# soedinglab/plass

Hardware: AMD Instinct MI355X
Metric: read-overlaps/s per assembly iteration (higher is better)
Workload: dtype u8/u64 (integer hash, byte compare; f32 ratios)

## Files before the change

plass_amd/csrc/kmermatch.hip:

```cpp
#include "common.hpp"
#include "device_utils.hpp"
#include "host_util.hpp"
#include "linepart.hpp"
#include "xxh64_u64.hpp"
#include <algorithm>
#include <memory>
#include <type_traits>
#include <cstdlib>
#include <climits>
#include <cstring>

namespace plasship {

#include "kmermatch_extract.hpp"
#include "kmermatch_group.hpp"
#include "kmermatch_repsort.hpp"
}
using namespace plasship;

namespace {

struct Timer {
    plasship_ctx *ctx; int slot;
    void start(int s) { slot = s; (void) hipEventRecord(ctx->ev[s], ctx->stream); }
// ... 58 lines not shown
    const uint64_t want = (lines + 4ull * (uint64_t) numCU - 1) / (4ull * (uint64_t) numCU);
    return (uint32_t) std::max<uint64_t>((uint64_t) nb * minFactor, std::min<uint64_t>((uint64_t) nb * 64, std::max<uint64_t>(want, 1)));
}
static LineGeo lineGeometry(uint64_t totalSlots, bool lng, int numCU, uint64_t slotsAll = 0, int W = 1) {
    LineGeo g;
    const int maxBits = lng ? 9 : 10;
    const int lw = ceilLog2((uint64_t) std::max(W, 1));
    const int totalBits = std::min(2 * maxBits, std::max(lw, std::max(0, ceilLog2(((slotsAll ? slotsAll : totalSlots) + 1535) / 1536))));
    g.b1 = totalBits <= maxBits ? totalBits : std::max((totalBits + 1) / 2, lw); g.b2 = totalBits - g.b1;
    g.nb1 = 1u << g.b1; g.nb2 = g.b2 ? 1u << g.b2 : 0u;
    g.totalLines = (totalSlots + RPL - 1) / RPL;
    g.lastValid = g.totalLines ? (uint32_t) (totalSlots - (g.totalLines - 1) * RPL) : (uint32_t) RPL;
    g.PL1 = pieceLinesFor(g.totalLines, g.nb1, numCU, 8);
    g.nP1 = (g.totalLines + g.PL1 - 1) / g.PL1;
    g.cap1 = std::max<uint64_t>(g.nP1 * ((uint64_t) g.PL1 + g.nb1), 1);
    if (g.nb2) {
        g.PL2 = 0xFFFFFFFFu; g.maxP2 = g.nb1; g.cap2 = g.cap1 + (uint64_t) g.nb1 * g.nb2;
    }
    return g;
}
static uint64_t repLevel1Cap(uint64_t nRec, uint64_t nSeg, uint32_t PL, uint32_t nb) {
    const uint64_t lines = (nRec + RPL - 1) / RPL + nSeg;
    return lines + (lines / PL + nSeg + 1) * (uint64_t) nb;
}

__global__ void arenaStartKernel(const uint32_t *__restrict__ lineBeg, uint32_t bpb, uint32_t gGrid, uint32_t nBuckets, uint64_t *__restrict__ arenaStart) {
    for (uint32_t j = blockIdx.x * blockDim.x + threadIdx.x; j < gGrid; j += gridDim.x * blockDim.x)
        arenaStart[j] = (uint64_t) lineBeg[std::min(j * bpb, nBuckets - 1)] * RPL;
}
__global__ void bigNeedKernel(const uint32_t *__restrict__ lineCnt, const uint32_t *__restrict__ unique, uint32_t nBuckets, uint64_t *__restrict__ need, uint32_t wordsPerEntry) {
    for (uint32_t b = blockIdx.x * blockDim.x + threadIdx.x; b < nBuckets; b += gridDim.x * blockDim.x) {
        const uint64_t c = (uint64_t) lineCnt[b] * RPL;
        uint64_t v = 0;
        if (unique[b] == AGG_NEEDS_SCRATCH) { uint64_t P = 1; while (P < c) P <<= 1; v = wordsPerEntry * P; }
        need[b] = v;
    }
}
__global__ void sumU32Kernel(const uint32_t *__restrict__ v, uint32_t n, unsigned long long *__restrict__ out) {
    unsigned long long s = 0;
    for (uint32_t i = blockIdx.x * blockDim.x + threadIdx.x; i < n; i += gridDim.x * blockDim.x) s += v[i];
    s = waveReduceSumU64(s);
    if (laneId() == 0 && s) atomicAdd(out, s);
}

template <class K> static int setDynLds(K k, size_t bytes) {
    PH_CHECK(hipFuncSetAttribute(reinterpret_cast<const void *>(k), hipFuncAttributeMaxDynamicSharedMemorySize, (int) bytes));
    return PLASSHIP_OK;
}
template <bool NUCL, bool LONG, int MODE, bool LIST, bool EXTRAS>
static int launchLinePart(plasship_ctx *ctx, const LinePartArgs &a, uint64_t nPiecesBound) {
    const size_t lds = linePartLdsBytes(a.nb, sizeof(Rec<LONG>), EXTRAS);
    const bool big = lds > 72 * 1024;
    const unsigned grid = (unsigned) std::max<uint64_t>(1, std::min<uint64_t>(nPiecesBound, (uint64_t) ctx->numCU * (big ? 1u : 2u)));
    if (big) {
        auto k = linePartKernel<NUCL, LONG, MODE, LIST, EXTRAS, 1024, 4, true>;
        const int rc = setDynLds(k, lds); if (rc) return rc;
        hipLaunchKernelGGL(k, dim3(grid), dim3(1024), lds, ctx->stream, a);
    } else {
        auto k = linePartKernel<NUCL, LONG, MODE, LIST, EXTRAS, 512, 4, true>;
        const int rc = setDynLds(k, lds); if (rc) return rc;
        hipLaunchKernelGGL(k, dim3(grid), dim3(512), lds, ctx->stream, a);
    }
    return PLASSHIP_OK;
}

static int buildLineLists(plasship_ctx *ctx, const uint32_t *dTags, uint64_t capLines, uint32_t nb, uint32_t *dCount, uint32_t *dStart, uint32_t *dCursor, uint32_t *dList) {
    hipStream_t st = ctx->stream;
    PH_CHECK(hipMemsetAsync(dCount, 0, (size_t) nb * 4, st));
    const unsigned g = (unsigned) std::max<uint64_t>(1, std::min<uint64_t>((capLines + 4095) / 4096, (uint64_t) ctx->numCU * 8));
    const unsigned gs = (unsigned) std::max<uint64_t>(1, std::min<uint64_t>((capLines + TS_CHUNK - 1) / TS_CHUNK, (uint64_t) ctx->numCU * 2));
    hipLaunchKernelGGL(tagHistKernel, dim3(g), dim3(256), 0, st, dTags, capLines, nb, dCount);
    hipLaunchKernelGGL(tagScanKernel, dim3(1), dim3(1024), 0, st, (const uint32_t *) dCount, nb, dStart, dCursor);
    hipLaunchKernelGGL(tagScatterKernel, dim3(gs), dim3(TS_BLOCK), 0, st, dTags, capLines, nb, dCursor, dList);
    return PLASSHIP_OK;
}

static bool shardOwnerFiltered(int W) { const int m = tuneInt("SHARD_EXTRACT", 0); return m == 2 || (m != 1 && W <= 4); }

constexpr int KM_RETRY_EARLY_OVERFLOW_CHECK = -1000;
struct LinesOut { void *triples = nullptr; uint64_t nTriples = 0, Nk = 0, Nm = 0; std::vector<int64_t> stalePos; uint32_t staleT = 0; float msSort1 = 0, msGroup = 0, msSort2 = 0, msPart = 0; int nPart = 1;
                  uint64_t exchangedRecordBytes = 0, exchangedTripleBytes = 0; };

constexpr uint64_t HALO_SLACK = 1u << 16;

template <bool NUCL, bool LONG, bool TRIPLES, bool ORDOUT = false>
static int repSortLines(plasship_ctx *ctx, const void *in, const std::vector<std::pair<uint64_t, uint64_t>> &segs, uint64_t nIn, uint32_t nReps, uint32_t repBase, uint32_t nTargets,
                        uint64_t slackTriples, const std::function<void()> &inputConsumed, DevBuf &dOut, uint64_t &nTriples, DevBuf *dRepStartOut) {
    constexpr bool PL = TRIPLES ? NUCL : LONG;
    typedef Rec<PL> R;
    typedef typename std::conditional<ORDOUT, TripleX, Triple>::type OutT;
    hipStream_t st = ctx->stream;
    const int numCU = ctx->numCU;
    const int maxBits = PL ? 9 : 10;
    const int idBits = std::max(1, ceilLog2((uint64_t) nTargets));
    const int repBits = std::max(1, ceilLog2((uint64_t) std::max<uint32_t>(nReps, 1)));
    const int wantBits = std::min(2 * maxBits, std::max(0, ceilLog2((nIn + 511) / 512)));
    const int allowedLocal = 62 - idBits - DiagPack<LONG>::BITS;
    const int sBits = std::max(std::min(wantBits, repBits), std::max(0, repBits - allowedLocal));
    if (sBits > 2 * maxBits) { setError("kmermatch: too many sequences for the packed rep-sort key"); return PLASSHIP_ERR_UNSUPPORTED; }
    const int s1 = sBits <= maxBits ? sBits : (sBits + 1) / 2, s2 = sBits - s1;
    const uint32_t nS1 = 1u << s1, nS2 = s2 ? 1u << s2 : 0u, nSort = 1u << sBits;
    std::vector<LinePiece> hp; uint64_t outLine = 0;
    {
        uint64_t totLines = 0; for (const auto &sg : segs) totLines += (sg.second + RPL - 1) / RPL;
        const uint32_t PLr1 = pieceLinesFor(totLines, nS1, numCU, 8);
        for (const auto &sg : segs) {
            const uint64_t cnt = sg.second, lines = (cnt + RPL - 1) / RPL;
            for (uint64_t l0 = 0; l0 < lines; l0 += PLr1) {
                LinePiece pc; pc.in0 = sg.first + l0; pc.nLines = (uint32_t) std::min<uint64_t>(PLr1, lines - l0);
                pc.lastValid = (l0 + pc.nLines == lines) ? (uint32_t) (cnt - (lines - 1) * RPL) : (uint32_t) RPL;
                pc.out0 = outLine; pc.outCap = pc.nLines + nS1; pc.tagBase = 0;
                outLine += pc.outCap; hp.push_back(pc);
            }
        }
    }
    const uint32_t PLr2 = s2 ? pieceLinesFor(std::max<uint64_t>(outLine, 1), nS2, numCU, 16) : 0;
    const uint64_t maxPR2 = s2 ? std::max<uint64_t>(outLine, 1) / PLr2 + nS1 + 1 : 0;
    const uint64_t capR1 = std::max<uint64_t>(outLine, 1), capR2 = s2 ? capR1 + maxPR2 * nS2 : 0;
    const uint32_t nPR1 = (uint32_t) hp.size();
    DevBuf dR1, dRTag1, dRList1, dRPieces, dRNP, dRCnt1, dRStart1, dRCur1, dR2, dRTag2, dRList2, dRPieces2, dRNP2, dRRegBeg, dRRegEnd, dRTot2, dSortBeg, dSortCnt;
    if (dR1.alloc(capR1 * RPL * sizeof(R)) != hipSuccess || dRTag1.alloc(capR1 * 4) != hipSuccess || dRList1.alloc(capR1 * 4) != hipSuccess || dRPieces.alloc(((size_t) nPR1 + 1) * sizeof(LinePiece)) != hipSuccess ||
        dRNP.alloc(4) != hipSuccess || dRCnt1.alloc(LP_MAXB * 4) != hipSuccess || dRStart1.alloc((LP_MAXB + 1) * 4) != hipSuccess || dRCur1.alloc(LP_MAXB * 4) != hipSuccess ||
        dSortBeg.alloc((size_t) nSort * 4) != hipSuccess || dSortCnt.alloc((size_t) nSort * 4) != hipSuccess) { setError("kmermatch: out of device memory for the rep sort"); return PLASSHIP_ERR_DEVICE; }
    void *hpPinned = nPR1 ? ctxPinnedTable(ctx, (size_t) nPR1 * sizeof(LinePiece)) : nullptr;
    if (hpPinned) memcpy(hpPinned, hp.data(), (size_t) nPR1 * sizeof(LinePiece));
    if (nPR1) PH_CHECK(hipMemcpyAsync(dRPieces.p, hpPinned ? hpPinned : (const void *) hp.data(), (size_t) nPR1 * sizeof(LinePiece), hipMemcpyHostToDevice, st));
    else PH_CHECK(hipMemsetAsync(dRTag1.p, 0xFF, capR1 * 4, st));
    PH_CHECK(hipMemcpyAsync(dRNP.p, &nPR1, 4, hipMemcpyHostToDevice, st));
    static const int directLines = [] { const char *e = getenv("PLASSHIP_DIRECT_LINES"); return e ? atoi(e) : 1; }();
    LineKey rkey; rkey.rangeBits = repBits; rkey.repBase = repBase; rkey.shift = s1 ? 64 - s1 : 63; rkey.scrambleBits = repBits;
    int rc;
    {
        LinePartArgs a; memset(&a, 0, sizeof(a));
        a.in = in; a.out = dR1.p; a.tags = dRTag1.as<uint32_t>(); a.pieces = dRPieces.as<LinePiece>(); a.nPieces = dRNP.as<uint32_t>(); a.nb = nS1; a.key = rkey;
        a.direct = directLines;
        rc = launchLinePart<NUCL, PL, KEY_RANGE, false, false>(ctx, a, std::max<uint32_t>(nPR1, 1)); if (rc) return rc;
    }
    if (nPR1 && !hpPinned) PH_CHECK(plasship::streamSync(st));
    rc = buildLineLists(ctx, dRTag1.as<uint32_t>(), capR1, nS1, dRCnt1.as<uint32_t>(), dRStart1.as<uint32_t>(), dRCur1.as<uint32_t>(), dRList1.as<uint32_t>()); if (rc) return rc;
    inputConsumed();
    const void *sortRecs = dR1.p; const uint32_t *sortList = dRList1.as<uint32_t>(); uint64_t sortCap = capR1;
    if (s2) {
        if (dR2.alloc(capR2 * RPL * sizeof(R)) != hipSuccess || dRTag2.alloc(capR2 * 4) != hipSuccess || dRList2.alloc(capR2 * 4) != hipSuccess || dRPieces2.alloc(((size_t) maxPR2 + 1) * sizeof(LinePiece)) != hipSuccess ||
            dRNP2.alloc(4) != hipSuccess || dRRegBeg.alloc(LP_MAXB * 8) != hipSuccess || dRRegEnd.alloc(LP_MAXB * 8) != hipSuccess || dRTot2.alloc(8) != hipSuccess) { setError("kmermatch: out of device memory for the rep sort"); return PLASSHIP_ERR_DEVICE; }
        hipLaunchKernelGGL(planListKernel, dim3(1), dim3(1024), 0, st, (const uint32_t *) dRStart1.as<uint32_t>(), nS1, PLr2, nS2, dRPieces2.as<LinePiece>(), dRNP2.as<uint32_t>(),
                           dRRegBeg.as<uint64_t>(), dRRegEnd.as<uint64_t>(), dRTot2.as<uint64_t>());
        LinePartArgs a; memset(&a, 0, sizeof(a));
        a.in = dR1.p; a.list = dRList1.as<uint32_t>(); a.out = dR2.p; a.tags = dRTag2.as<uint32_t>(); a.pieces = dRPieces2.as<LinePiece>(); a.nPieces = dRNP2.as<uint32_t>(); a.nb = nS2;
        a.direct = directLines;
        a.key = rkey; a.key.shift = 64 - s1 - s2;
        rc = launchLinePart<NUCL, PL, KEY_RANGE, true, false>(ctx, a, maxPR2); if (rc) return rc;
        hipLaunchKernelGGL(tagSortRegionKernel, dim3(std::min<uint32_t>(nS1, (uint32_t) numCU * 4)), dim3(512), 0, st, (const uint32_t *) dRTag2.as<uint32_t>(), (const uint64_t *) dRRegBeg.as<uint64_t>(),
                           (const uint64_t *) dRRegEnd.as<uint64_t>(), nS1, nS2, dRList2.as<uint32_t>(), dSortBeg.as<uint32_t>(), dSortCnt.as<uint32_t>());
        sortRecs = dR2.p; sortList = dRList2.as<uint32_t>(); sortCap = capR2;
    } else {
        hipLaunchKernelGGL(listRangesKernel, dim3(4), dim3(256), 0, st, (const uint32_t *) dRStart1.as<uint32_t>(), nS1, dSortBeg.as<uint32_t>(), dSortCnt.as<uint32_t>());
    }
    DevBuf dBigNeed, dBigOff, dBigScratch, dUnique, dScanTmp3, dSparse;
    const size_t scanTmp3Bytes = exclusiveScanTmpBytes((size_t) nSort + 2);
    if (dBigNeed.alloc(((size_t) nSort + 1) * 8) != hipSuccess || dBigOff.alloc(((size_t) nSort + 2) * 8) != hipSuccess || dUnique.alloc(((size_t) nSort + 1) * 4) != hipSuccess ||
        dScanTmp3.alloc(scanTmp3Bytes) != hipSuccess || dSparse.alloc(sortCap * RPL * sizeof(OutT)) != hipSuccess) {
        setError("kmermatch: out of device memory for the rep sort"); return PLASSHIP_ERR_DEVICE;
    }
    const AggLines aggLn{sortList, dSortBeg.as<uint32_t>(), dSortCnt.as<uint32_t>()};
    const unsigned aggGrid = std::min<uint32_t>(nSort, (uint32_t) numCU * (uint32_t) tuneInt("AGGSORT", 16));
    hipLaunchKernelGGL((aggSortKernel<NUCL, LONG, true, TRIPLES, ORDOUT>), dim3(aggGrid), dim3(LS_BLOCK), 0, st, sortRecs, dSparse.p, (const uint64_t *) nullptr, nSort,
                       (unsigned long long *) nullptr, (const uint64_t *) nullptr, dUnique.as<uint32_t>(), repBits - sBits, idBits, (uint64_t) repBase, aggLn, repBits);
    hipLaunchKernelGGL(bigNeedKernel, dim3(gridFor(nSort, 256, 1024)), dim3(256), 0, st, (const uint32_t *) dSortCnt.as<uint32_t>(), (const uint32_t *) dUnique.as<uint32_t>(), nSort, dBigNeed.as<uint64_t>(), NUCL ? 3u : 2u);
    if (exclusiveScanU64(st, dBigNeed.as<uint64_t>(), dBigOff.as<uint64_t>(), nSort, dScanTmp3.p, scanTmp3Bytes)) { setError("kmermatch: scan failed"); return PLASSHIP_ERR_DEVICE; }
    uint64_t bigTot = 0;
    PH_COPY_SYNC(st, &bigTot, dBigOff.as<uint64_t>() + nSort, 8, hipMemcpyDeviceToHost);
    PH_CHECK(hipGetLastError());
    if (bigTot) {
        if (dBigScratch.alloc(bigTot * 8) != hipSuccess) { setError("kmermatch: out of device memory for the rep sort"); return PLASSHIP_ERR_DEVICE; }
        hipLaunchKernelGGL((aggSortKernel<NUCL, LONG, true, TRIPLES, ORDOUT>), dim3(aggGrid), dim3(LS_BLOCK), 0, st, sortRecs, dSparse.p, (const uint64_t *) nullptr, nSort,
                           dBigScratch.as<unsigned long long>(), (const uint64_t *) dBigOff.as<uint64_t>(), dUnique.as<uint32_t>(), repBits - sBits, idBits, (uint64_t) repBase, aggLn, repBits);
    }
    DevBuf dRepCnt, dRepStartLocal, dScanTmp4;
    DevBuf &dRepStart = dRepStartOut ? *dRepStartOut : dRepStartLocal;
    const size_t scanTmp4Bytes = exclusiveScanTmpBytes((size_t) nReps + 2);
    if (dRepCnt.alloc(((size_t) nReps + 1) * 4) != hipSuccess || dRepStart.alloc(((size_t) nReps + 2) * 8) != hipSuccess ||
        dScanTmp4.alloc(scanTmp4Bytes) != hipSuccess) { setError("kmermatch: out of device memory for the rep sort"); return PLASSHIP_ERR_DEVICE; }
    PH_CHECK(hipMemsetAsync(dRepCnt.p, 0, ((size_t) nReps + 1) * 4, st));
    const unsigned runGrid = std::min<uint32_t>((nSort + 3) / 4, (uint32_t) numCU * 8);
    hipLaunchKernelGGL(repRunsKernel<OutT>, dim3(runGrid), dim3(256), 0, st, (const OutT *) dSparse.p, (const uint32_t *) dSortBeg.as<uint32_t>(),
                       (const uint32_t *) dUnique.as<uint32_t>(), nSort, repBase, dRepCnt.as<uint32_t>());
    if (exclusiveScanU32(st, dRepCnt.as<uint32_t>(), dRepStart.as<uint64_t>(), nReps, dScanTmp4.p, scanTmp4Bytes)) { setError("kmermatch: scan failed"); return PLASSHIP_ERR_DEVICE; }
    nTriples = 0;
    PH_COPY_SYNC(st, &nTriples, dRepStart.as<uint64_t>() + nReps, 8, hipMemcpyDeviceToHost);
    PH_CHECK(hipGetLastError());
    dR1.release(); dR2.release();
    if (dOut.alloc((std::max<uint64_t>(nTriples, 1) + slackTriples) * sizeof(OutT)) != hipSuccess) { setError("kmermatch: out of device memory for the sorted triples"); return PLASSHIP_ERR_DEVICE; }
    if (nTriples) hipLaunchKernelGGL(placeRunsKernel<OutT>, dim3(runGrid), dim3(256), 0, st, (const OutT *) dSparse.p, (const uint32_t *) dSortBeg.as<uint32_t>(), (const uint32_t *) dUnique.as<uint32_t>(), nSort,
                                     repBase, (const uint64_t *) dRepStart.as<uint64_t>(), (OutT *) dOut.p);
    PH_CHECK(hipGetLastError());
    return PLASSHIP_OK;
}

static void moveBuf(DevBuf &dst, DevBuf &src) { dst.release(); dst.p = src.p; dst.bytes = src.bytes; src.p = nullptr; src.bytes = 0; }

template <bool NUCL, bool LONG>
static int kmermatchLines(plasship_ctx *ctx, const plasship_seqdb *db, const plasship_kmermatch_params *par, const LineGeo &geo, uint64_t total,
                          DevBuf &dA, DevBuf &dB, const DevBuf &dSlotOff, const DevBuf &dKStats, const ExtractArgs &ea, int keyBits, LinesOut &res,
                          const uint32_t *dLateOverflow, bool filtered) {
    typedef Rec<LONG> R;
    hipStream_t st = ctx->stream;
    const uint32_t N = (uint32_t) db->n;
    const int numCU = ctx->numCU;
    const plasship_comm *cm = commOf(ctx);
    const int W = cm ? cm->world : 1, rk = cm ? cm->rank : 0;
    const bool exch = cm && !filtered;
    const int valueShift = std::max(0, keyBits - 11);
    PH_CHECK(hipEventRecord(ctx->ev[1], st));
    const uint32_t bLo = cm ? (uint32_t) ownedBegin(geo.nb1, rk, W) : 0u, bHi = cm ? (uint32_t) ownedBegin(geo.nb1, rk + 1, W) : geo.nb1;
    const uint32_t nbL = bHi - bLo;
    DevBuf dVHist, dMinKey, dTag1, dList1, dCnt1, dStart1, dCur1, dTag2, dList2, dPieces2, dNP2, dRegBeg, dRegEnd, dTot2, dFineBeg, dFineCnt;
    DevBuf dRx, dRxList, dRxSegs, dRxStart;
    const uint32_t nBuckets = geo.nb2 ? nbL * geo.nb2 : nbL;
    if (dVHist.alloc(VH_BINS * 4) != hipSuccess || dMinKey.alloc(8) != hipSuccess || dTag1.alloc(geo.cap1 * 4) != hipSuccess || dList1.alloc(geo.cap1 * 4) != hipSuccess ||
        dCnt1.alloc(LP_MAXB * 4) != hipSuccess || dStart1.alloc((LP_MAXB + 1) * 4) != hipSuccess || dCur1.alloc(LP_MAXB * 4) != hipSuccess ||
        dFineBeg.alloc((size_t) std::max<uint32_t>(nBuckets, 1) * 4) != hipSuccess || dFineCnt.alloc((size_t) std::max<uint32_t>(nBuckets, 1) * 4) != hipSuccess ||
        (geo.nb2 && (dPieces2.alloc((geo.maxP2 + 1) * sizeof(LinePiece)) != hipSuccess ||
                     dNP2.alloc(4) != hipSuccess || dRegBeg.alloc(LP_MAXB * 8) != hipSuccess || dRegEnd.alloc(LP_MAXB * 8) != hipSuccess || dTot2.alloc(8) != hipSuccess))) {
        setError("kmermatch: out of device memory for the line lists"); return PLASSHIP_ERR_DEVICE;
    }
    PH_CHECK(hipMemsetAsync(dVHist.p, 0, VH_BINS * 4, st));
    PH_CHECK(hipMemsetAsync(dMinKey.p, 0xFF, 8, st));
    if (geo.nP1 == 0) PH_CHECK(hipMemsetAsync(dTag1.p, 0xFF, geo.cap1 * 4, st));
    {
        LinePartArgs a; memset(&a, 0, sizeof(a));
        a.in = dA.p; a.out = dB.p; a.tags = dTag1.as<uint32_t>(); a.totalLines = geo.totalLines; a.lastValidAll = geo.lastValid; a.pieceLines = geo.PL1; a.nb = geo.nb1;
        a.key.shift = geo.b1 ? 64 - geo.b1 : 63; a.key.rangeBits = 0; a.key.repBase = 0;
        a.minKey = NUCL ? dMinKey.as<unsigned long long>() : nullptr; a.valueHist = dVHist.as<uint32_t>(); a.valueShift = valueShift;
        if (cm && filtered) { a.keepLo = bLo; a.keepHi = bHi; }
        PH_CHECK(hipEventRecord(ctx->ev[8], st));
        const int rc = launchLinePart<NUCL, LONG, KEY_HASH, false, true>(ctx, a, geo.nP1); if (rc) return rc;
        PH_CHECK(hipEventRecord(ctx->ev[9], st));
    }
    int rc = buildLineLists(ctx, dTag1.as<uint32_t>(), geo.cap1, geo.nb1, dCnt1.as<uint32_t>(), dStart1.as<uint32_t>(), dCur1.as<uint32_t>(), dList1.as<uint32_t>()); if (rc) return rc;
    void *l1Recs = dB.p; const uint32_t *l1List = dList1.as<uint32_t>(); const uint32_t *l1Start = dStart1.as<uint32_t>() + bLo; uint64_t l1Lines = geo.cap1;
    const uint32_t *l1Tags = dTag1.as<uint32_t>();
    uint64_t NkAll = 0;
    if (cm && filtered && NUCL) {
        uint64_t mk = 0; PH_COPY_SYNC(st, &mk, dMinKey.p, 8, hipMemcpyDeviceToHost);
        rc = commAllReduceMinU64(ctx, &mk, 1); if (rc) return rc;
        PH_COPY_SYNC(st, dMinKey.p, &mk, 8, hipMemcpyHostToDevice);
    }
    if (exch) {
        std::vector<uint32_t> hStart1(geo.nb1 + 1);
        PH_COPY_SYNC(st, hStart1.data(), dStart1.p, ((size_t) geo.nb1 + 1) * 4, hipMemcpyDeviceToHost);
        PH_CHECK(hipGetLastError());
        const uint64_t myLines = hStart1[geo.nb1];
        const uint64_t selfBeg = hStart1[ownedBegin(geo.nb1, rk, W)], selfEnd = hStart1[ownedBegin(geo.nb1, rk + 1, W)];
        const uint64_t selfLines = selfEnd - selfBeg, sendLines = myLines - selfLines;
        const uint32_t chunksPerLine = (uint32_t) (RPL * sizeof(R) / 16);
        auto gather = [&](uint64_t listFrom, uint64_t n, void *dst) {
            if (n) hipLaunchKernelGGL(gatherLinesKernel, dim3(gridFor(n * chunksPerLine, 256, (unsigned) numCU * 16)), dim3(256), 0, st, (const uint4 *) dB.p, (const uint32_t *) dList1.as<uint32_t>() + listFrom,
                                      n, chunksPerLine, (uint4 *) dst);
        };
        dA.release();
        if (dA.alloc(std::max<uint64_t>(sendLines, 1) * RPL * sizeof(R)) != hipSuccess) { setError("kmermatch: out of device memory for the send buffer"); return PLASSHIP_ERR_DEVICE; }
        gather(0, selfBeg, dA.p);
        gather(selfEnd, myLines - selfEnd, (char *) dA.p + selfBeg * RPL * sizeof(R));
        dTag1.release();
        std::vector<uint64_t> mine((size_t) geo.nb1 + 1), all(((size_t) geo.nb1 + 1) * (size_t) W);
        for (uint32_t j = 0; j < geo.nb1; j++) mine[j] = hStart1[j + 1] - hStart1[j];
        { unsigned long long ks[4] = {0, 0, 0, 0}; PH_COPY_SYNC(st, ks, dKStats.p, 32, hipMemcpyDeviceToHost); mine[geo.nb1] = ks[1] + ks[3]; }
        rc = commAllgatherHost(ctx, mine.data(), all.data(), mine.size() * 8); if (rc) return rc;
        std::vector<uint64_t> sendCount(W);
// ... 653 lines not shown
```

plass_amd/csrc/kmermatch_repsort.hpp:

```cpp
#pragma once

constexpr int LS_BLOCK = 256;
constexpr uint32_t AGG_CAP = 1024;
constexpr uint32_t AGG_HT = 2048;
constexpr uint32_t AGG_NEEDS_SCRATCH = 0xFFFFFFFFu;
template <bool LONG> struct DiagPack { static constexpr int BITS = LONG ? 22 : 16; static constexpr int64_t BIAS = LONG ? (1 << 21) : 32768; };
struct __attribute__((aligned(16))) Triple { uint32_t rep, target; int32_t diag; uint32_t cnt; };
struct __attribute__((aligned(8))) TripleX { uint32_t rep, target; int32_t diag; uint32_t cnt; uint64_t ord; };
static_assert(sizeof(TripleX) == sizeof(Rec<true>) && sizeof(Triple) == sizeof(Rec<false>), "triples travel through the line store as records");

struct AggLines { const uint32_t *list, *lineBeg, *lineCnt; };
__device__ __forceinline__ bool isSentinel(const Triple &t) { return t.rep == 0xFFFFFFFFu && t.target == 0xFFFFFFFFu; }
__device__ __forceinline__ bool isSentinel(const TripleX &t) { return t.rep == 0xFFFFFFFFu && t.target == 0xFFFFFFFFu; }
template <bool NUCL, bool LONG, bool LINES, bool TRIPLES = false, bool ORDOUT = false>
__global__ __launch_bounds__(LS_BLOCK) void aggSortKernel(const void *arr, void *outTriples, const uint64_t *__restrict__ bucketStart, uint32_t nBuckets,
                                                          unsigned long long *bigScratch, const uint64_t *__restrict__ bigOff,
                                                          uint32_t *__restrict__ uniqueCount, int localBits, int idBits, uint64_t repBase, AggLines ln, int scrambleBits) {
    static_assert(!ORDOUT || NUCL, "only nucleotide triples carry a strand");
    typedef typename std::conditional<TRIPLES, typename std::conditional<NUCL, TripleX, Triple>::type, Rec<LONG>>::type R;
    typedef typename std::conditional<ORDOUT, TripleX, Triple>::type O;
    __shared__ unsigned long long hKey[AGG_HT];
    __shared__ uint32_t hVal[AGG_HT];
    __shared__ unsigned long long hOrd[NUCL ? AGG_HT : 1];
    __shared__ unsigned long long lKey[AGG_CAP];
    __shared__ uint32_t lVal[AGG_CAP];
    __shared__ unsigned long long lOrd[NUCL ? AGG_CAP : 1];
    __shared__ uint32_t sCount;
    __shared__ uint32_t sDistinct, sOver;
    __shared__ uint32_t sWave[LS_BLOCK / 64];
    const R *g = reinterpret_cast<const R *>(arr);
    O *out = reinterpret_cast<O *>(outTriples);
    constexpr int DB = DiagPack<LONG>::BITS;
    for (uint32_t b = blockIdx.x; b < nBuckets; b += gridDim.x) {
        const uint64_t s0 = LINES ? (uint64_t) ln.lineBeg[b] * RPL : bucketStart[b];
        const uint64_t cnt = LINES ? (uint64_t) ln.lineCnt[b] * RPL : bucketStart[b + 1] - s0;
        const uint32_t lb = LINES ? ln.lineBeg[b] : 0u;
        auto recAt = [&](uint64_t i) -> R { if (LINES) return g[(uint64_t) ln.list[lb + (uint32_t) (i / RPL)] * RPL + (i % RPL)]; return g[s0 + i]; };
        if (cnt == 0) { if (threadIdx.x == 0) uniqueCount[b] = 0; continue; }
        const uint64_t bucketBase = (uint64_t) b << localBits;
        auto decode = [&](unsigned long long key, uint32_t val, unsigned long long ord) {
            O t;
            t.diag = (int32_t) ((int64_t) (key & ((1ULL << DB) - 1)) - DiagPack<LONG>::BIAS);
            const uint64_t k2 = key >> DB;
            t.target = (uint32_t) (k2 & ((1ULL << idBits) - 1));
            const uint64_t rp = (k2 >> idBits) + bucketBase;
            t.rep = (uint32_t) ((scrambleBits ? scrambleRep(rp, scrambleBits) : rp) + repBase);
            t.cnt = val;
            if constexpr (ORDOUT) t.ord = ord;
            return t;
        };
        auto packRec = [&](const R &r, uint32_t &val, unsigned long long &ord) {
            uint64_t rep, target; int64_t diag; ord = 0;
            if constexpr (TRIPLES) { rep = r.rep; target = r.target; diag = r.diag; val = r.cnt & 0x7FFFFFFFu; if constexpr (NUCL) ord = r.ord; }
            else { rep = (uint32_t) r.kmer; target = r.id; diag = r.pos; val = 1u; if constexpr (NUCL) ord = ordWordOf(r); }
            rep -= repBase;
            if (scrambleBits) rep = scrambleRep(rep, scrambleBits);
            return (unsigned long long) (((((rep - bucketBase) << idBits) | target) << DB) | (uint64_t) (diag + DiagPack<LONG>::BIAS));
        };
        auto clearTable = [&]() {
            for (uint32_t i = threadIdx.x; i < AGG_HT; i += LS_BLOCK) { hKey[i] = ~0ULL; hVal[i] = 0; if (NUCL) hOrd[i] = 0; }
            if (threadIdx.x == 0) sCount = 0;
            __syncthreads();
        };
        auto insert = [&](unsigned long long key, uint32_t val, unsigned long long ord) {
            uint32_t slot = (uint32_t) ((key * 0x9E3779B97F4A7C15ULL) >> 40) & (AGG_HT - 1);
            for (;;) {
                const unsigned long long prev = atomicCAS(&hKey[slot], ~0ULL, key);
                if (prev == ~0ULL || prev == key) break;
                slot = (slot + 1) & (AGG_HT - 1);
            }
            atomicAdd(&hVal[slot], val);
            if (NUCL) atomicMax(&hOrd[slot], ord);
        };
        auto extract = [&]() {
            for (uint32_t i = threadIdx.x; i < AGG_HT; i += LS_BLOCK) {
                const unsigned long long k = hKey[i];
                if (k != ~0ULL) {
                    const uint32_t o = atomicAdd(&sCount, 1u); lKey[o] = k;
                    if (NUCL) { const unsigned long long od = hOrd[i]; lOrd[o] = od; lVal[o] = hVal[i] | ((uint32_t) (od & 1ULL) << 31); }
                    else lVal[o] = hVal[i];
                }
            }
            __syncthreads();
            return sCount;
        };
        auto sortListAndWrite = [&](uint32_t U) {
            uint32_t P = 1; while (P < U) P <<= 1;
            for (uint32_t i = U + threadIdx.x; i < P; i += LS_BLOCK) { lKey[i] = ~0ULL; lVal[i] = 0; if (ORDOUT) lOrd[i] = 0; }
            __syncthreads();
            for (uint32_t kk = 2; kk <= P; kk <<= 1) {
                for (uint32_t j = kk >> 1; j > 0; j >>= 1) {
                    for (uint32_t t = threadIdx.x; t < (P >> 1); t += LS_BLOCK) {
                        const uint32_t i = ((t & ~(j - 1)) << 1) | (t & (j - 1));
                        const uint32_t l = i | j;
                        const unsigned long long x = lKey[i], y = lKey[l];
                        const bool up = (i & kk) == 0;
                        if ((x > y) == up) {
                            lKey[i] = y; lKey[l] = x; const uint32_t vx = lVal[i]; lVal[i] = lVal[l]; lVal[l] = vx;
                            if (ORDOUT) { const unsigned long long ox = lOrd[i]; lOrd[i] = lOrd[l]; lOrd[l] = ox; }
                        }
                    }
                    __syncthreads();
                }
            }
            for (uint32_t i = threadIdx.x; i < U; i += LS_BLOCK) out[s0 + i] = decode(lKey[i], lVal[i], ORDOUT ? lOrd[i] : 0ull);
            if (threadIdx.x == 0) uniqueCount[b] = U;
            __syncthreads();
        };
        if (bigScratch && uniqueCount[b] != AGG_NEEDS_SCRATCH) continue;
        bool done = false;
        if (!bigScratch && cnt <= (1ull << 22)) {
            clearTable();
            if (threadIdx.x == 0) { sDistinct = 0; sOver = 0; }
            __syncthreads();
            for (uint64_t i = threadIdx.x; i < cnt && !*(volatile uint32_t *) &sOver; i += LS_BLOCK) {
                const R r = recAt(i); if (LINES && isSentinel(r)) continue;
// ... 18 lines not shown
        if (!bigScratch) { if (threadIdx.x == 0) uniqueCount[b] = AGG_NEEDS_SCRATCH; continue; }
        {
            unsigned long long *pk = bigScratch + bigOff[b];
            uint64_t P0 = 1; while (P0 < cnt) P0 <<= 1;
            unsigned long long *pv = pk + P0, *po = pv + P0;
            uint64_t nPart = 0;
            for (uint64_t c0 = 0; c0 < cnt; c0 += AGG_CAP) {
                const uint64_t c1 = min(cnt, c0 + (uint64_t) AGG_CAP);
                clearTable();
                for (uint64_t i = c0 + threadIdx.x; i < c1; i += LS_BLOCK) { const R r = recAt(i); if (LINES && isSentinel(r)) continue; uint32_t v; unsigned long long od; const unsigned long long key = packRec(r, v, od); insert(key, v, od); }
                __syncthreads();
                const uint32_t U = extract();
                for (uint32_t i = threadIdx.x; i < U; i += LS_BLOCK) { pk[nPart + i] = lKey[i]; pv[nPart + i] = lVal[i] & 0x7FFFFFFFu; if (NUCL) po[nPart + i] = lOrd[i]; }
                nPart += U;
                __syncthreads();
            }
            bool fits = true;
            if (nPart <= (uint64_t) AGG_HT) {
                clearTable();
                for (uint64_t i = threadIdx.x; i < nPart; i += LS_BLOCK) insert(pk[i], (uint32_t) pv[i], NUCL ? po[i] : 0ull);
                __syncthreads();
                uint32_t mine = 0;
                for (uint32_t i = threadIdx.x; i < AGG_HT; i += LS_BLOCK) mine += (hKey[i] != ~0ULL) ? 1u : 0u;
                mine = (uint32_t) waveReduceSum((int) mine);
                if (laneId() == 0) sWave[threadIdx.x >> 6] = mine;
                __syncthreads();
                uint32_t tot = 0;
#pragma unroll
                for (int w = 0; w < LS_BLOCK / 64; w++) tot += sWave[w];
                __syncthreads();
                fits = tot <= AGG_CAP;
                if (fits) sortListAndWrite(extract());
            } else fits = false;
            if (!fits) {
                uint64_t P = 1; while (P < nPart) P <<= 1;
                for (uint64_t i = nPart + threadIdx.x; i < P; i += LS_BLOCK) { pk[i] = ~0ULL; pv[i] = 0; if (NUCL) po[i] = 0; }
                __syncthreads();
                for (uint64_t kk = 2; kk <= P; kk <<= 1) {
                    for (uint64_t j = kk >> 1; j > 0; j >>= 1) {
                        for (uint64_t t = threadIdx.x; t < (P >> 1); t += LS_BLOCK) {
                            const uint64_t i = ((t & ~(j - 1)) << 1) | (t & (j - 1));
                            const uint64_t l = i | j;
                            const unsigned long long x = pk[i], y = pk[l];
                            const bool up = (i & kk) == 0;
                            if ((x > y) == up) {
                                pk[i] = y; pk[l] = x; const unsigned long long vx = pv[i]; pv[i] = pv[l]; pv[l] = vx;
                                if (NUCL) { const unsigned long long ox = po[i]; po[i] = po[l]; po[l] = ox; }
                            }
                        }
                        __syncthreads();
                    }
                }
                uint32_t written = 0;
                for (uint64_t i0 = 0; i0 < nPart; i0 += LS_BLOCK) {
                    const uint64_t i = i0 + threadIdx.x;
                    bool head = false; O t; t.rep = t.target = t.cnt = 0; t.diag = 0;
                    if (i < nPart) {
                        const unsigned long long k = pk[i];
                        head = (i == 0) || (pk[i - 1] != k);
                        if (head) {
                            uint32_t c = 0; unsigned long long om = 0;
                            for (uint64_t j = i; j < nPart && pk[j] == k; j++) { c += (uint32_t) pv[j]; if (NUCL) om = max(om, po[j]); }
                            t = decode(k, c | ((uint32_t) (om & 1ULL) << 31), om);
                        }
                    }
                    const unsigned long long mk = __ballot(head);
                    const uint32_t wr = (uint32_t) __popcll(mk & ((1ULL << laneId()) - 1ULL));
                    if (laneId() == 0) sWave[threadIdx.x >> 6] = (uint32_t) __popcll(mk);
                    __syncthreads();
                    uint32_t woff = 0, tot = 0;
#pragma unroll
                    for (int w = 0; w < LS_BLOCK / 64; w++) { if (w < (int) (threadIdx.x >> 6)) woff += sWave[w]; tot += sWave[w]; }
                    if (head) out[s0 + written + woff + wr] = t;
                    written += tot;
                    __syncthreads();
                }
                if (threadIdx.x == 0) uniqueCount[b] = written;
                __syncthreads();
            }
        }
    }
}

template <class T>
__global__ __launch_bounds__(256) void repRunsKernel(const T *__restrict__ in, const uint32_t *__restrict__ lineBeg, const uint32_t *__restrict__ unique, uint32_t nBuckets,
                                                     uint32_t repBase, uint32_t *__restrict__ cnt) {
    for (uint32_t b = blockIdx.x * 4 + (threadIdx.x >> 6); b < nBuckets; b += gridDim.x * 4) {
        const uint64_t s0 = (uint64_t) lineBeg[b] * RPL; const uint32_t n = unique[b];
        for (uint32_t i0 = 0; i0 < n; i0 += 64) {
            const uint32_t i = i0 + laneId();
            const bool valid = i < n;
            const uint32_t rep = valid ? in[s0 + i].rep : 0xFFFFFFFFu;
            const uint32_t prevLane = __shfl_up(rep, 1, 64);
            const bool segHead = valid && (laneId() == 0 || prevLane != rep);
            const unsigned long long heads = __ballot(segHead), vmask = __ballot(valid);
            if (segHead) {
                const unsigned long long later = heads & ~((2ULL << laneId()) - 1ULL);
                const int end = later ? __ffsll((long long) later) - 1 : (int) __popcll(vmask);
                atomicAdd(&cnt[rep - repBase], (uint32_t) (end - laneId()));
            }
        }
    }
}
template <class T>
__global__ __launch_bounds__(256) void placeRunsKernel(const T *__restrict__ in, const uint32_t *__restrict__ lineBeg, const uint32_t *__restrict__ unique, uint32_t nBuckets,
                                                       uint32_t repBase, const uint64_t *__restrict__ start, T *__restrict__ out) {
    const int lane = laneId();
    for (uint32_t b = blockIdx.x * 4 + (threadIdx.x >> 6); b < nBuckets; b += gridDim.x * 4) {
        const uint64_t s0 = (uint64_t) lineBeg[b] * RPL; const uint32_t n = unique[b];
        uint32_t carryRep = 0xFFFFFFFFu, carryHead = 0;
        for (uint32_t i0 = 0; i0 < n; i0 += 64) {
            const uint32_t i = i0 + (uint32_t) lane;
            const bool valid = i < n;
            T t; t.rep = 0xFFFFFFFFu; t.target = 0; t.diag = 0; t.cnt = 0;
            if (valid) t = in[s0 + i];
            const uint32_t rep = t.rep;
            const uint32_t prevLane = __shfl_up(rep, 1, 64);
            const bool segHead = valid && (lane == 0 || prevLane != rep);
            const unsigned long long heads = __ballot(segHead), vmask = __ballot(valid);
            const unsigned long long below = heads & ((lane == 63) ? ~0ULL : ((2ULL << lane) - 1ULL));
            const int headLane = 63 - __clzll((long long) below);
            const uint32_t rep0 = (uint32_t) __shfl((int) rep, 0, 64);
            const uint32_t runHead = (headLane == 0 && rep0 == carryRep) ? carryHead : i0 + (uint32_t) headLane;
            if (valid) out[start[rep - repBase] + (uint64_t) (i - runHead)] = t;
            const int lastLane = (int) __popcll(vmask) - 1;
            carryRep = (uint32_t) __shfl((int) rep, lastLane, 64); carryHead = (uint32_t) __shfl((int) runHead, lastLane, 64);
        }
    }
}
__global__ void ownerBoundsKernel(const uint64_t *__restrict__ start, uint64_t n, int W, uint64_t *__restrict__ out) {
    for (int r = threadIdx.x; r <= W; r += blockDim.x) out[r] = start[((uint64_t) r * n + (uint64_t) W - 1) / (uint64_t) W];
}
__global__ __launch_bounds__(256) void gatherLinesKernel(const uint4 *__restrict__ in, const uint32_t *__restrict__ list, uint64_t nLines, uint32_t chunksPerLine, uint4 *__restrict__ out) {
    const uint64_t total = nLines * chunksPerLine;
    for (uint64_t i = (uint64_t) blockIdx.x * blockDim.x + threadIdx.x; i < total; i += (uint64_t) gridDim.x * blockDim.x)
        out[i] = in[(uint64_t) list[i / chunksPerLine] * chunksPerLine + (i % chunksPerLine)];
}
struct RxSeg { uint64_t src; uint32_t cnt, dst; };
__global__ __launch_bounds__(256) void rxListKernel(const RxSeg *__restrict__ segs, uint32_t nSegs, uint32_t *__restrict__ list) {
    for (uint32_t q = blockIdx.x; q < nSegs; q += gridDim.x) { const RxSeg g = segs[q]; for (uint32_t i = threadIdx.x; i < g.cnt; i += 256) list[g.dst + i] = (uint32_t) (g.src + i); }
}

template <bool NUCL>
__global__ __launch_bounds__(256) void reduceRunsKernel(const Triple *__restrict__ h, uint64_t n, uint64_t nScan, CandHit *__restrict__ tmpHits, uint32_t *__restrict__ emitW,
                                 uint32_t *__restrict__ perRep) {
    const int lane = threadIdx.x & 63;
    for (uint64_t i = (uint64_t) blockIdx.x * blockDim.x + threadIdx.x; i < n; i += (uint64_t) gridDim.x * blockDim.x) {
        const Triple r = h[i];
        bool head = (i == 0);
        if (!head) { const Triple q = h[i - 1]; head = (q.rep != r.rep) || (q.target != r.target); }
        uint32_t e = 0;
        CandHit c; c.target = 0; c.prefScore = 0; c.diag16 = 0; c.query = 0;
        if (head) {
            const uint32_t targetId = r.target;
            int32_t diagonal = r.diag, prevDiagonal = r.diag;
            uint64_t maxDiagonal = 0, diagonalCnt = 0, topScore = 0;
            int bestRev = NUCL ? ((r.cnt & 0x80000000u) == 0) : 0;
            for (uint64_t j = i; j < nScan; j++) {
                const Triple x = h[j];
                if (x.target != targetId) break;
                const uint64_t cc = x.cnt & 0x7FFFFFFFu;
                if (prevDiagonal == x.diag) diagonalCnt += cc; else diagonalCnt = cc;
                if (diagonalCnt >= maxDiagonal) { diagonal = x.diag; maxDiagonal = diagonalCnt; if (NUCL) bestRev = ((x.cnt & 0x80000000u) == 0); }
                prevDiagonal = x.diag; topScore += cc;
            }
            if (targetId != r.rep) {
                c.target = targetId; c.prefScore = bestRev ? -(int) topScore : (int) topScore;
                c.diag16 = (uint32_t) (uint16_t) diagonal; c.query = r.rep;
                e = 1;
            }
// ... 65 lines not shown
```

Before: 685.3 million.

## Add wave-per-bucket LDS hash aggregation with overflow list for rep sort

```diff
diff --git a/plass_amd/csrc/kmermatch.hip b/plass_amd/csrc/kmermatch.hip
--- a/plass_amd/csrc/kmermatch.hip
+++ b/plass_amd/csrc/kmermatch.hip
@@ -164,6 +164,29 @@
                   uint64_t exchangedRecordBytes = 0, exchangedTripleBytes = 0; };
 
 constexpr uint64_t HALO_SLACK = 1u << 16;
+
+static bool aggHistOn() { return getenv("PLASSHIP_DEBUG_AGGHIST") != nullptr; }
+static int aggHistRecord(hipStream_t st, const uint32_t *dLineCnt, const uint32_t *dUnique, uint32_t nSort) {
+    static int call = 0;
+    std::vector<uint32_t> lc(nSort), uq(nSort);
+    PH_COPY_SYNC(st, lc.data(), dLineCnt, (size_t) nSort * 4, hipMemcpyDeviceToHost);
+    PH_COPY_SYNC(st, uq.data(), dUnique, (size_t) nSort * 4, hipMemcpyDeviceToHost);
+    constexpr int NB = 10;
+    auto bin = [](uint64_t v) { if (!v) return 0; int k = 1; uint64_t e = 64; while (k < NB - 1 && v > e) { e <<= 1; k++; } return k; };
+    uint64_t hr[NB] = {}, hd[NB] = {}, sr = 0, sd = 0, mr = 0, md = 0, big = 0;
+    for (uint32_t b = 0; b < nSort; b++) {
+        const uint64_t r = (uint64_t) lc[b] * RPL; hr[bin(r)]++; sr += r; mr = std::max(mr, r);
+        if (uq[b] == AGG_NEEDS_SCRATCH) { big++; continue; }
+        hd[bin(uq[b])]++; sd += uq[b]; md = std::max<uint64_t>(md, uq[b]);
+    }
+    std::string s = "aggHist call " + std::to_string(call++) + " buckets " + std::to_string(nSort) + " | bins 0,<=64,<=128,...,<=8192,>8192 | slots";
+    for (int k = 0; k < NB; k++) s += " " + std::to_string(hr[k]);
+    s += " (mean " + std::to_string(nSort ? sr / nSort : 0) + ", max " + std::to_string(mr) + ") | distinct";
+    for (int k = 0; k < NB; k++) s += " " + std::to_string(hd[k]);
+    s += " (mean " + std::to_string(nSort ? sd / nSort : 0) + ", max " + std::to_string(md) + ", scratch " + std::to_string(big) + ")";
+    fprintf(stderr, "%s\n", s.c_str());
+    return PLASSHIP_OK;
+}
 
 template <bool NUCL, bool LONG, bool TRIPLES, bool ORDOUT = false>
 static int repSortLines(plasship_ctx *ctx, const void *in, const std::vector<std::pair<uint64_t, uint64_t>> &segs, uint64_t nIn, uint32_t nReps, uint32_t repBase, uint32_t nTargets,
@@ -244,10 +267,31 @@
         dScanTmp3.alloc(scanTmp3Bytes) != hipSuccess || dSparse.alloc(sortCap * RPL * sizeof(OutT)) != hipSuccess) {
         setError("kmermatch: out of device memory for the rep sort"); return PLASSHIP_ERR_DEVICE;
     }
+    DevBuf dRepCnt, dRepStartLocal, dScanTmp4;
+    DevBuf &dRepStart = dRepStartOut ? *dRepStartOut : dRepStartLocal;
+    const size_t scanTmp4Bytes = exclusiveScanTmpBytes((size_t) nReps + 2);
+    if (dRepCnt.alloc(((size_t) nReps + 1) * 4) != hipSuccess || dRepStart.alloc(((size_t) nReps + 2) * 8) != hipSuccess ||
+        dScanTmp4.alloc(scanTmp4Bytes) != hipSuccess) { setError("kmermatch: out of device memory for the rep sort"); return PLASSHIP_ERR_DEVICE; }
+    PH_CHECK(hipMemsetAsync(dRepCnt.p, 0, ((size_t) nReps + 1) * 4, st));
+    const bool aggWave = tuneInt("AGGWAVE", 1) != 2;
     const AggLines aggLn{sortList, dSortBeg.as<uint32_t>(), dSortCnt.as<uint32_t>()};
     const unsigned aggGrid = std::min<uint32_t>(nSort, (uint32_t) numCU * (uint32_t) tuneInt("AGGSORT", 16));
+    DevBuf dOver;
+    const uint32_t *ovList = nullptr, *ovCount = nullptr;
+    if (aggWave) {
+        if (dOver.alloc(((size_t) nSort + 1) * 4) != hipSuccess) { setError("kmermatch: out of device memory for the rep sort"); return PLASSHIP_ERR_DEVICE; }
+        PH_CHECK(hipMemsetAsync(dOver.p, 0, 4, st));
+        const uint32_t capT = (uint32_t) tuneInt("AGGWAVE_CAP", (int) AW_CAP);
+        AggWaveArgs wa; wa.capKeys = std::min<uint32_t>(capT, AW_CAP); wa.capRecs = std::min<uint32_t>(AW_RECS, wa.capKeys * 16u);
+        wa.ovCount = dOver.as<uint32_t>(); wa.ovList = wa.ovCount + 1; wa.repCnt = dRepCnt.as<uint32_t>();
+        ovCount = wa.ovCount; ovList = wa.ovList;
+        constexpr int WPB = AggWaveGeo<NUCL>::WPB;
+        const unsigned wGrid = std::min<uint32_t>((nSort + WPB - 1) / WPB, (uint32_t) numCU * (uint32_t) tuneInt("AGGWAVE_GRID", (int) AggWaveGeo<NUCL>::PER_CU));
+        hipLaunchKernelGGL((aggSortWaveKernel<NUCL, LONG, TRIPLES, ORDOUT>), dim3(wGrid), dim3(WPB * 64), 0, st, sortRecs, dSparse.p, nSort, dUnique.as<uint32_t>(),
+                           repBits - sBits, idBits, (uint64_t) repBase, aggLn, repBits, wa);
+    }
     hipLaunchKernelGGL((aggSortKernel<NUCL, LONG, true, TRIPLES, ORDOUT>), dim3(aggGrid), dim3(LS_BLOCK), 0, st, sortRecs, dSparse.p, (const uint64_t *) nullptr, nSort,
-                       (unsigned long long *) nullptr, (const uint64_t *) nullptr, dUnique.as<uint32_t>(), repBits - sBits, idBits, (uint64_t) repBase, aggLn, repBits);
+                       (unsigned long long *) nullptr, (const uint64_t *) nullptr, dUnique.as<uint32_t>(), repBits - sBits, idBits, (uint64_t) repBase, aggLn, repBits, ovList, ovCount);
     hipLaunchKernelGGL(bigNeedKernel, dim3(gridFor(nSort, 256, 1024)), dim3(256), 0, st, (const uint32_t *) dSortCnt.as<uint32_t>(), (const uint32_t *) dUnique.as<uint32_t>(), nSort, dBigNeed.as<uint64_t>(), NUCL ? 3u : 2u);
     if (exclusiveScanU64(st, dBigNeed.as<uint64_t>(), dBigOff.as<uint64_t>(), nSort, dScanTmp3.p, scanTmp3Bytes)) { setError("kmermatch: scan failed"); return PLASSHIP_ERR_DEVICE; }
     uint64_t bigTot = 0;
@@ -256,17 +300,13 @@
     if (bigTot) {
         if (dBigScratch.alloc(bigTot * 8) != hipSuccess) { setError("kmermatch: out of device memory for the rep sort"); return PLASSHIP_ERR_DEVICE; }
         hipLaunchKernelGGL((aggSortKernel<NUCL, LONG, true, TRIPLES, ORDOUT>), dim3(aggGrid), dim3(LS_BLOCK), 0, st, sortRecs, dSparse.p, (const uint64_t *) nullptr, nSort,
-                           dBigScratch.as<unsigned long long>(), (const uint64_t *) dBigOff.as<uint64_t>(), dUnique.as<uint32_t>(), repBits - sBits, idBits, (uint64_t) repBase, aggLn, repBits);
-    }
-    DevBuf dRepCnt, dRepStartLocal, dScanTmp4;
-    DevBuf &dRepStart = dRepStartOut ? *dRepStartOut : dRepStartLocal;
-    const size_t scanTmp4Bytes = exclusiveScanTmpBytes((size_t) nReps + 2);
-    if (dRepCnt.alloc(((size_t) nReps + 1) * 4) != hipSuccess || dRepStart.alloc(((size_t) nReps + 2) * 8) != hipSuccess ||
-        dScanTmp4.alloc(scanTmp4Bytes) != hipSuccess) { setError("kmermatch: out of device memory for the rep sort"); return PLASSHIP_ERR_DEVICE; }
-    PH_CHECK(hipMemsetAsync(dRepCnt.p, 0, ((size_t) nReps + 1) * 4, st));
+                           dBigScratch.as<unsigned long long>(), (const uint64_t *) dBigOff.as<uint64_t>(), dUnique.as<uint32_t>(), repBits - sBits, idBits, (uint64_t) repBase, aggLn, repBits,
+                           ovList, ovCount);
+    }
+    if (aggHistOn()) { const int hrc = aggHistRecord(st, dSortCnt.as<uint32_t>(), dUnique.as<uint32_t>(), nSort); if (hrc) return hrc; }
     const unsigned runGrid = std::min<uint32_t>((nSort + 3) / 4, (uint32_t) numCU * 8);
     hipLaunchKernelGGL(repRunsKernel<OutT>, dim3(runGrid), dim3(256), 0, st, (const OutT *) dSparse.p, (const uint32_t *) dSortBeg.as<uint32_t>(),
-                       (const uint32_t *) dUnique.as<uint32_t>(), nSort, repBase, dRepCnt.as<uint32_t>());
+                       (const uint32_t *) dUnique.as<uint32_t>(), nSort, repBase, dRepCnt.as<uint32_t>(), ovList, ovCount);
     if (exclusiveScanU32(st, dRepCnt.as<uint32_t>(), dRepStart.as<uint64_t>(), nReps, dScanTmp4.p, scanTmp4Bytes)) { setError("kmermatch: scan failed"); return PLASSHIP_ERR_DEVICE; }
     nTriples = 0;
     PH_COPY_SYNC(st, &nTriples, dRepStart.as<uint64_t>() + nReps, 8, hipMemcpyDeviceToHost);
diff --git a/plass_amd/csrc/kmermatch_repsort.hpp b/plass_amd/csrc/kmermatch_repsort.hpp
--- a/plass_amd/csrc/kmermatch_repsort.hpp
+++ b/plass_amd/csrc/kmermatch_repsort.hpp
@@ -15,7 +15,8 @@
 template <bool NUCL, bool LONG, bool LINES, bool TRIPLES = false, bool ORDOUT = false>
 __global__ __launch_bounds__(LS_BLOCK) void aggSortKernel(const void *arr, void *outTriples, const uint64_t *__restrict__ bucketStart, uint32_t nBuckets,
                                                           unsigned long long *bigScratch, const uint64_t *__restrict__ bigOff,
-                                                          uint32_t *__restrict__ uniqueCount, int localBits, int idBits, uint64_t repBase, AggLines ln, int scrambleBits) {
+                                                          uint32_t *__restrict__ uniqueCount, int localBits, int idBits, uint64_t repBase, AggLines ln, int scrambleBits,
+                                                          const uint32_t *__restrict__ bList = nullptr, const uint32_t *__restrict__ bListN = nullptr) {
     static_assert(!ORDOUT || NUCL, "only nucleotide triples carry a strand");
     typedef typename std::conditional<TRIPLES, typename std::conditional<NUCL, TripleX, Triple>::type, Rec<LONG>>::type R;
     typedef typename std::conditional<ORDOUT, TripleX, Triple>::type O;
@@ -31,7 +32,9 @@
     const R *g = reinterpret_cast<const R *>(arr);
     O *out = reinterpret_cast<O *>(outTriples);
     constexpr int DB = DiagPack<LONG>::BITS;
-    for (uint32_t b = blockIdx.x; b < nBuckets; b += gridDim.x) {
+    const uint32_t nB = bList ? *bListN : nBuckets;
+    for (uint32_t q = blockIdx.x; q < nB; q += gridDim.x) {
+        const uint32_t b = bList ? bList[q] : q;
         const uint64_t s0 = LINES ? (uint64_t) ln.lineBeg[b] * RPL : bucketStart[b];
         const uint64_t cnt = LINES ? (uint64_t) ln.lineCnt[b] * RPL : bucketStart[b + 1] - s0;
         const uint32_t lb = LINES ? ln.lineBeg[b] : 0u;
@@ -216,10 +219,222 @@
     }
 }
 
+constexpr uint32_t AW_CAP = 512;
+constexpr uint32_t AW_RECS = 8192;
+constexpr int AW_LOADS = 4;
+template <bool NUCL> struct AggWaveGeo {
+    static constexpr uint32_t HT = 2 * AW_CAP;
+    static constexpr int WPB = NUCL ? 2 : 4;
+    static constexpr uint32_t LDS = WPB * (HT * (NUCL ? 20u : 12u) + AW_CAP * 8u);
+    static constexpr uint32_t PER_CU = (160u * 1024u) / LDS;
+};
+struct AggWaveArgs { uint32_t capKeys, capRecs; uint32_t *ovList, *ovCount; uint32_t *repCnt; };
+
+__device__ __forceinline__ void waveFence() { __builtin_amdgcn_fence(__ATOMIC_ACQ_REL, "wavefront"); __builtin_amdgcn_wave_barrier(); }
+template <int J> __device__ __forceinline__ unsigned long long xorLane64(unsigned long long v) {
+    if constexpr (J == 1) return dppMov64<0xB1>(v);
+    else if constexpr (J == 2) return dppMov64<0x4E>(v);
+    else if constexpr (J < 32) {
+        const uint32_t lo = (uint32_t) __builtin_amdgcn_ds_swizzle((int) (uint32_t) v, 0x1F | (J << 10));
+        const uint32_t hi = (uint32_t) __builtin_amdgcn_ds_swizzle((int) (uint32_t) (v >> 32), 0x1F | (J << 10));
+        return ((unsigned long long) hi << 32) | lo;
+    } else return __shfl_xor(v, J, 64);
+}
+template <int EB, int E> __device__ __forceinline__ void waveBitonic(unsigned long long (&k)[E]) {
+    const int lane = laneId();
+#pragma unroll
+    for (int kk = 2; kk <= 64 * EB; kk <<= 1) {
+#pragma unroll
+        for (int j = kk >> 1; j > 0; j >>= 1) {
+            if (j >= 64) {
+                const int je = j >> 6;
+#pragma unroll
+                for (int e = 0; e < EB; e++)
+                    if ((e & je) == 0) {
+                        const bool up = ((e << 6) & kk) == 0;
+                        const unsigned long long x = k[e], y = k[e | je];
+                        const bool sw = (x > y) == up;
+                        k[e] = sw ? y : x; k[e | je] = sw ? x : y;
+                    }
+            } else {
+#pragma unroll
+                for (int e = 0; e < EB; e++) {
+                    unsigned long long y;
+                    switch (j) { case 1: y = xorLane64<1>(k[e]); break; case 2: y = xorLane64<2>(k[e]); break; case 4: y = xorLane64<4>(k[e]); break;
+                                 case 8: y = xorLane64<8>(k[e]); break; case 16: y = xorLane64<16>(k[e]); break; default: y = xorLane64<32>(k[e]); }
+                    const bool up = ((((e << 6) | lane) & kk) == 0), low = (lane & j) == 0;
+                    const unsigned long long mn = k[e] < y ? k[e] : y, mx = k[e] < y ? y : k[e];
+                    k[e] = (low == up) ? mn : mx;
+                }
+            }
+        }
+    }
+}
+
+template <bool NUCL, bool LONG, bool TRIPLES = false, bool ORDOUT = false>
+__global__ __launch_bounds__(AggWaveGeo<NUCL>::WPB * 64) void aggSortWaveKernel(const void *arr, void *outTriples, uint32_t nBuckets, uint32_t *__restrict__ uniqueCount,
+                                                                                 int localBits, int idBits, uint64_t repBase, AggLines ln, int scrambleBits, AggWaveArgs wa) {
+    static_assert(!ORDOUT || NUCL, "only nucleotide triples carry a strand");
+    typedef typename std::conditional<TRIPLES, typename std::conditional<NUCL, TripleX, Triple>::type, Rec<LONG>>::type R;
+    typedef typename std::conditional<ORDOUT, TripleX, Triple>::type O;
+    constexpr uint32_t HT = AggWaveGeo<NUCL>::HT;
+    constexpr int WPB = AggWaveGeo<NUCL>::WPB, E = AW_CAP / 64;
+    constexpr int DB = DiagPack<LONG>::BITS;
+    __shared__ unsigned long long sKey[WPB][HT];
+    __shared__ uint32_t sVal[WPB][HT];
+    __shared__ unsigned long long sOrd[NUCL ? WPB : 1][NUCL ? HT : 1];
+    __shared__ unsigned long long sList[WPB][AW_CAP];
+    const int wv = (int) (threadIdx.x >> 6), lane = laneId();
+    unsigned long long *hKey = sKey[wv], *hOrd = sOrd[NUCL ? wv : 0], *lKey = sList[wv];
+    uint32_t *hVal = sVal[wv];
+    const R *g = reinterpret_cast<const R *>(arr);
+    O *out = reinterpret_cast<O *>(outTriples);
+    for (uint32_t i = lane; i < HT; i += 64) { hKey[i] = ~0ULL; hVal[i] = 0; if (NUCL) hOrd[i] = 0; }
+    waveFence();
+    const uint32_t nW = gridDim.x * WPB;
+    struct Lines { uint32_t lb, lc, le0, le1; };
+    auto fetchLines = [&](uint32_t bb) {
+        Lines L; L.lb = ln.lineBeg[bb]; L.lc = ln.lineCnt[bb];
+        L.le0 = (uint32_t) lane < L.lc ? ln.list[L.lb + lane] : 0u;
+        L.le1 = (uint32_t) lane + 64 < L.lc ? ln.list[L.lb + 64 + lane] : 0u;
+        return L;
+    };
+    auto loadBatch = [&](const Lines &L, uint32_t i0, R (&r)[AW_LOADS]) {
+#pragma unroll
+        for (int u = 0; u < AW_LOADS; u++) {
+            const uint32_t i = i0 + (uint32_t) (u * 64 + lane), line = i / RPL;
+            const uint32_t a0 = (uint32_t) __shfl((int) L.le0, (int) (line & 63), 64), a1 = (uint32_t) __shfl((int) L.le1, (int) (line & 63), 64);
+            if (i < L.lc * RPL) { const uint32_t le = line < 64 ? a0 : line < 128 ? a1 : ln.list[L.lb + line]; r[u] = g[(uint64_t) le * RPL + (i % RPL)]; }
+        }
+    };
+    uint32_t b = blockIdx.x * WPB + (uint32_t) wv;
+    Lines cur = {0u, 0u, 0u, 0u};
+    R r[AW_LOADS];
+    if (b < nBuckets) { cur = fetchLines(b); loadBatch(cur, 0, r); }
+    for (; b < nBuckets; b += nW) {
+        const uint32_t lb = (uint32_t) __builtin_amdgcn_readfirstlane((int) cur.lb), lc = (uint32_t) __builtin_amdgcn_readfirstlane((int) cur.lc);
+        cur.lb = lb; cur.lc = lc;
+        const bool more = b + nW < nBuckets;
+        Lines nxt = {0u, 0u, 0u, 0u};
+        if (more) nxt = fetchLines(b + nW);
+        const uint32_t cnt = lc * RPL;
+        const uint64_t s0 = (uint64_t) lb * RPL;
+        const uint64_t bucketBase = (uint64_t) b << localBits;
+        auto packRec = [&](const R &r, uint32_t &val, unsigned long long &ord) {
+            uint64_t rep, target; int64_t diag; ord = 0;
+            if constexpr (TRIPLES) { rep = r.rep; target = r.target; diag = r.diag; val = r.cnt & 0x7FFFFFFFu; if constexpr (NUCL) ord = r.ord; }
+            else { rep = (uint32_t) r.kmer; target = r.id; diag = r.pos; val = 1u; if constexpr (NUCL) ord = ordWordOf(r); }
+            rep -= repBase;
+            if (scrambleBits) rep = scrambleRep(rep, scrambleBits);
+            return (unsigned long long) (((((rep - bucketBase) << idBits) | target) << DB) | (uint64_t) (diag + DiagPack<LONG>::BIAS));
+        };
+        bool over = cnt > wa.capRecs;
+        uint32_t U = 0;
+        for (uint32_t i0 = 0; i0 < cnt && !over; i0 += 64 * AW_LOADS) {
+            const bool pre = i0 + 64 * AW_LOADS < cnt;
+            R rn[AW_LOADS];
+            if (pre) loadBatch(cur, i0 + 64 * AW_LOADS, rn);
+#pragma unroll
+            for (int u = 0; u < AW_LOADS; u++) {
+                bool fresh = false;
+                if (i0 + (uint32_t) (u * 64 + lane) < cnt && !isSentinel(r[u])) {
+                    uint32_t v; unsigned long long od; const unsigned long long key = packRec(r[u], v, od);
+                    uint32_t slot = (uint32_t) ((key * 0x9E3779B97F4A7C15ULL) >> 40) & (HT - 1);
+                    for (;;) {
+                        const unsigned long long prev = atomicCAS(&hKey[slot], ~0ULL, key);
+                        if (prev == ~0ULL) { fresh = true; break; }
+                        if (prev == key) break;
+                        slot = (slot + 1) & (HT - 1);
+                    }
+                    atomicAdd(&hVal[slot], v);
+                    if (NUCL) atomicMax(&hOrd[slot], od);
+                }
+                U += (uint32_t) __popcll(__ballot(fresh));
+                if (U > wa.capKeys) { over = true; break; }
+            }
+            if (pre) {
+#pragma unroll
+                for (int u = 0; u < AW_LOADS; u++) r[u] = rn[u];
+            }
+        }
+        if (more) { cur = nxt; loadBatch(cur, 0, r); }
+        waveFence();
+        if (over) {
+            if (U) { for (uint32_t i = lane; i < HT; i += 64) { hKey[i] = ~0ULL; hVal[i] = 0; if (NUCL) hOrd[i] = 0; } waveFence(); }
+            if (lane == 0) wa.ovList[atomicAdd(wa.ovCount, 1u)] = b;
+            continue;
+        }
+        if (U == 0) { if (lane == 0) uniqueCount[b] = 0; continue; }
+        uint32_t n = 0;
+        for (uint32_t s = 0; s < HT; s += 64) {
+            const unsigned long long kx = hKey[s + lane];
+            const bool occ = kx != ~0ULL;
+            const unsigned long long m = __ballot(occ);
+            if (occ) lKey[n + (uint32_t) __popcll(m & ((1ULL << lane) - 1ULL))] = kx;
+            n += (uint32_t) __popcll(m);
+        }
+        waveFence();
+        unsigned long long k[E];
+#pragma unroll
+        for (int e = 0; e < E; e++) { const uint32_t i = (uint32_t) (e * 64 + lane); k[e] = i < U ? lKey[i] : ~0ULL; }
+        const uint32_t nE = (U + 63) / 64;
+        if (nE <= 1) waveBitonic<1>(k);
+        else if (nE <= 2) waveBitonic<2>(k);
+        else if (nE <= 4) waveBitonic<4>(k);
+        else waveBitonic<8>(k);
+        const int RS = DB + idBits;
+        unsigned long long hm[E];
+        uint64_t prevTop = __shfl(k[0] >> RS, 0, 64);
+#pragma unroll
+        for (int e = 0; e < E; e++) {
+            const uint32_t i = (uint32_t) (e * 64 + lane);
+            const uint64_t rp = k[e] >> RS, up = __shfl_up(rp, 1, 64);
+            const bool head = i < U && (i == 0 || (lane ? up : prevTop) != rp);
+            hm[e] = __ballot(head);
+            prevTop = __shfl(rp, 63, 64);
+        }
+        uint32_t after[E];
+        uint32_t nh = U;
+#pragma unroll
+        for (int e = E - 1; e >= 0; e--) { after[e] = nh; if (hm[e]) nh = (uint32_t) (e * 64) + (uint32_t) (__ffsll((long long) hm[e]) - 1); }
+#pragma unroll
+        for (int e = 0; e < E; e++) {
+            const uint32_t i = (uint32_t) (e * 64 + lane);
+            if ((uint32_t) (e * 64) >= U) break;
+            if (i < U) {
+                const unsigned long long key = k[e];
+                uint32_t slot = (uint32_t) ((key * 0x9E3779B97F4A7C15ULL) >> 40) & (HT - 1);
+                while (hKey[slot] != key) slot = (slot + 1) & (HT - 1);
+                uint32_t val = hVal[slot]; unsigned long long od = 0;
+                if (NUCL) { od = hOrd[slot]; val |= (uint32_t) (od & 1ULL) << 31; hOrd[slot] = 0; }
+                hKey[slot] = ~0ULL; hVal[slot] = 0;
+                O t;
+                t.diag = (int32_t) ((int64_t) (key & ((1ULL << DB) - 1)) - DiagPack<LONG>::BIAS);
+                const uint64_t k2 = key >> DB;
+                t.target = (uint32_t) (k2 & ((1ULL << idBits) - 1));
+                const uint64_t rp = (k2 >> idBits) + bucketBase;
+                t.rep = (uint32_t) ((scrambleBits ? scrambleRep(rp, scrambleBits) : rp) + repBase);
+                t.cnt = val;
+                if constexpr (ORDOUT) t.ord = od;
+                out[s0 + i] = t;
+                if ((hm[e] >> lane) & 1ULL) {
+                    const unsigned long long later = lane == 63 ? 0ULL : (hm[e] & ~((2ULL << lane) - 1ULL));
+                    const uint32_t end = later ? (uint32_t) (e * 64) + (uint32_t) (__ffsll((long long) later) - 1) : after[e];
+                    wa.repCnt[t.rep - (uint32_t) repBase] = end - i;
+                }
+            }
+        }
+        if (lane == 0) uniqueCount[b] = U;
+        waveFence();
+    }
+}
+
 template <class T>
 __global__ __launch_bounds__(256) void repRunsKernel(const T *__restrict__ in, const uint32_t *__restrict__ lineBeg, const uint32_t *__restrict__ unique, uint32_t nBuckets,
-                                                     uint32_t repBase, uint32_t *__restrict__ cnt) {
-    for (uint32_t b = blockIdx.x * 4 + (threadIdx.x >> 6); b < nBuckets; b += gridDim.x * 4) {
+                                                     uint32_t repBase, uint32_t *__restrict__ cnt, const uint32_t *__restrict__ bList, const uint32_t *__restrict__ bListN) {
+    const uint32_t nB = bList ? *bListN : nBuckets;
+    for (uint32_t q = blockIdx.x * 4 + (threadIdx.x >> 6); q < nB; q += gridDim.x * 4) {
+        const uint32_t b = bList ? bList[q] : q;
         const uint64_t s0 = (uint64_t) lineBeg[b] * RPL; const uint32_t n = unique[b];
         for (uint32_t i0 = 0; i0 < n; i0 += 64) {
             const uint32_t i = i0 + laneId();
```

Result: faster. 705.1 million, median of 6 (+2.9%).
